# UCSD-Comp-Imaging/Nerf-Simple

Hardware: AMD Instinct MI355X
Metric: ray-samples/sec at 800x800x128 (higher is better)
Workload: dtype f16

## Files before the change

### nerf-simple_amd/csrc/mlp_bf16_16.hip

```cpp
#include "composite_device.h"

using namespace nerf_layout;

#ifdef NERF_HALF
typedef _Float16 elem_t;
#define NERF_MFMA __builtin_amdgcn_mfma_f32_16x16x32_f16
#define NERF_KERNEL nerf_mlp_f16_16_kernel
#define NERF_LAUNCH nerf_amd_launch_mlp_f16_16
#else
typedef __bf16 elem_t;
#define NERF_MFMA __builtin_amdgcn_mfma_f32_16x16x32_bf16
#define NERF_KERNEL nerf_mlp_bf16_16_kernel
#define NERF_LAUNCH nerf_amd_launch_mlp_bf16_16
#endif
#include "mlp16_chain.h"

namespace {

#ifdef NERF_HALF
constexpr bool FOLD = true;
#else
constexpr bool FOLD = false;
#endif
struct MlpPlan {
    static constexpr int LAYERS = NUM_LAYERS;
    static constexpr bool SAVE = !FOLD;
    static constexpr int tpc(int L) { return L == 0 ? 8 : 4; }
    static constexpr int mt(int L) { return FOLD ? fold_mt(L) : b16_mt(L); }
    static constexpr int layer_off_kib(int L) { return FOLD ? fold_layer_off_kib(L) : b16_layer_off_kib(L); }
    static constexpr int bias_off(int L) { return FOLD ? fold_bias_off(L) : b16_bias_off(L); }
};
static_assert(NUM_CHUNKS<MlpPlan> == (FOLD ? 34 : 38) && plan_fits<MlpPlan>(), "chunks per tile / weight buffer, parity");

constexpr int LDS_POSD = LDS_CHAIN_END;
constexpr int LDS_POSX = LDS_POSD + WAVES * NCB * 1024;
constexpr int LDS_TOTAL = LDS_POSX + WAVES * NCB * 2048;
constexpr int RING_PTS = 1024;
constexpr int LDS_RING_RAW = LDS_TOTAL;
constexpr int LDS_RING_T = LDS_RING_RAW + RING_PTS * 16;
constexpr int LDS_TOTAL_COMP = LDS_RING_T + RING_PTS * 4;
constexpr int COMP_MAX_N = RING_PTS - TILE_PTS;
static_assert(COMP_MAX_N == FUSED_RENDER_MAX_N, "api.hip routes by this limit");
static_assert(LDS_TOTAL_COMP <= 160 * 1024, "LDS budget");
static_assert((RING_PTS & (RING_PTS - 1)) == 0 && RING_PTS % TILE_PTS == 0, "ring indexing");

static_assert(ACT_TILE_PTS == TILE_PTS && MASK_TILE_PTS == TILE_PTS, "activation blocks and mask tiles are the kernel's tiles");

struct State {
    using Plan = MlpPlan;
    ex8 X[NCB][8], Y[NCB][8];
    f32x4 pend[NCB][2];
    float sigma[NCB], rgb[NCB][3];
    bool bad;
    unsigned posd_off[NCB];
    char* acts;
    long long P;
    long long tile;
    int loff[NCB];
    unsigned mb[NCB][2];
    float amax[4];
    long long mask_tile;
    long long p_end;
    unsigned ring_q0;
    WFrag* wf;
};

template <bool RAYS, int SAVE, bool COMP>
__device__ __forceinline__ void stage_inputs(const Ctx& c, const MlpArgs& a, long long tile_base, State& st) {
    const int col = c.lane & 15, g = c.lane >> 4;
    float u_mine = 0.f;
    bool dev_rng = false;
    long long b0 = 0;
    int r0 = 0;
    if constexpr (RAYS) {
        b0 = tile_base / a.N;
        r0 = (int)(tile_base - b0 * a.N);
    }
    const long long p_end = COMP ? st.p_end : a.P;
    const int last_local = (int)(p_end - 1 - tile_base);
    constexpr bool RAY_POSD = RAYS && !SAVE;
    if constexpr (RAY_POSD) {
        const int top = last_local < TILE_PTS - 1 ? last_local : TILE_PTS - 1;
        const int nrays = (int)(split_point(b0, r0, top, a.N).b - b0) + 1;
        for (int idx = threadIdx.x; idx < nrays * 32; idx += WAVES * 64) {
            const int ray = idx >> 5, slot = idx & 31, gg = slot >> 3, sl = slot & 7;
            const float* rp = a.rays + (b0 + ray) * 6 + 3;
            const float dx = rp[0], dy = rp[1], dz = rp[2];
            const float nrm = norm3(dx, dy, dz);
            float val = 0.f;
            if (sl < 6) {
                const int cd = sl >> 1;
                const float dc = __fdiv_rn(cd == 0 ? dx : cd == 1 ? dy : dz, nrm);
                val = enc_lane(to_revolutions(dc), 2 * gg + (sl & 1));
            } else if (sl == 6 && gg < 3) {
                val = __fdiv_rn(gg == 0 ? dx : gg == 1 ? dy : dz, nrm);
            }
            lds_store<elem_t>(LDS_POSD + ray * 64 + slot * 2, 0, (elem_t)val);
        }
    }
    if constexpr (RAYS && NCB == 2) {
        dev_rng = (a.flags & NERF_FLAG_DEVICE_RNG) && !(a.flags & NERF_FLAG_TS_GIVEN);
        if (dev_rng) {
            int lm = c.wave * 32 + (c.lane & 31);
            if (lm > last_local) lm = last_local;
            u_mine = device_rng_uniform(a, split_point(b0, r0, lm, a.N));
        }
    }
#pragma unroll
    for (int cb = 0; cb < NCB; ++cb) {
        long long p = tile_base + c.wave * (16 * NCB) + cb * 16 + col;
        const bool valid = p < p_end;
        st.loff[cb] = valid ? block_lane_offset(g, c.wave * (16 * NCB) + cb * 16 + col) : LOFF_INVALID;
        if constexpr (SAVE == 2) {
            if (cb == 0)
                st.loff[0] = tile_base + c.wave * 32 + 16 * (c.lane >> 5) + col < p_end ? f8_lane_offset(c.lane, c.wave) : LOFF_INVALID;
        }
        if (!valid) p = p_end - 1;
        PointIn pt;
        st.posd_off[cb] = c.b_posd + cb * 1024;
        if constexpr (RAYS) {
            const float u_cb = (NCB == 2) ? __shfl(u_mine, cb * 16 + col) : 0.f;
            int lp = c.wave * (16 * NCB) + cb * 16 + col;
            if (lp > last_local) lp = last_local;
            if (SAVE && a.pts) {
                pt = fetch_point_pts(a, p);
            } else {
                const RaySample rs = split_point(b0, r0, lp, a.N);
                if constexpr (RAY_POSD) st.posd_off[cb] = LDS_POSD + (unsigned)(rs.b - b0) * 64 + g * 16;
                pt = fetch_point_rays<!RAY_POSD>(a, p, rs, u_cb, dev_rng);
                if constexpr (COMP) {
                    if (valid && g == 0)
                        lds_store<float>(((st.ring_q0 + c.wave * (16 * NCB) + cb * 16 + col) & (RING_PTS - 1)) * 4, LDS_RING_T, pt.t);
                }
                if (valid && g == 0 && a.ts_out) a.ts_out[p] = pt.t;
            }
        } else {
            pt = fetch_point_pts(a, p);
        }
        {
            const float xyz[3] = {pt.x, pt.y, pt.z};
            float v[16];
#pragma unroll
            for (int cd = 0; cd < 3; ++cd) {
                const TwoF q = to_revolutions(xyz[cd]);
#pragma unroll
                for (int jj = 0; jj < 5; ++jj) v[cd * 5 + jj] = enc_lane(q, 5 * g + jj);
            }
            v[15] = g == 0 ? pt.x : g == 1 ? pt.y : g == 2 ? pt.z : 0.f;
#pragma unroll
            for (int e = 0; e < 2; ++e) {
                u32x4 r;
#pragma unroll
                for (int i = 0; i < 4; ++i) r[i] = pack2<false>(v[8 * e + 2 * i], v[8 * e + 2 * i + 1]);
                lds_store<u32x4>(c.b_posx, cb * 2048 + e * 1024, r);
            }
        }
        if constexpr (!RAY_POSD) {
            const float dd[3] = {pt.d1, pt.d2, pt.d3};
            float v[8];
#pragma unroll
            for (int cd = 0; cd < 3; ++cd) {
                const TwoF q = to_revolutions(dd[cd]);
#pragma unroll
                for (int jj = 0; jj < 2; ++jj) v[cd * 2 + jj] = enc_lane(q, 2 * g + jj);
            }
            v[6] = g == 0 ? pt.d1 : g == 1 ? pt.d2 : g == 2 ? pt.d3 : 0.f;
            v[7] = 0.f;
            u32x4 r;
#pragma unroll
            for (int i = 0; i < 4; ++i) r[i] = pack2<false>(v[2 * i], v[2 * i + 1]);
            lds_store<u32x4>(c.b_posd, cb * 1024, r);
        }
    }
}

template <bool RAYS, int SAVE, bool COMP>
__device__ __forceinline__ void run_tile(const Ctx& c, const MlpArgs& a, long long tile_base, State& st) {
    stage_inputs<RAYS, SAVE, COMP>(c, a, tile_base, st);
    run_layer<0, SAVE>(c, st, st.X, st.X);
    run_layer<1, SAVE>(c, st, st.X, st.Y);
    run_layer<2, SAVE>(c, st, st.Y, st.X);
    run_layer<3, SAVE>(c, st, st.X, st.Y);
    run_layer<4, SAVE>(c, st, st.Y, st.X);
    run_layer<5, SAVE>(c, st, st.X, st.Y);
    run_layer<6, SAVE>(c, st, st.Y, st.X);
    run_layer<7, SAVE>(c, st, st.X, st.Y);
    ex8 (&c_in)[NCB][8] = FOLD ? st.Y : st.X;
    ex8 (&c_out)[NCB][8] = FOLD ? st.X : st.Y;
    run_layer<8, SAVE>(c, st, st.Y, st.X);
    run_layer<9, SAVE>(c, st, c_in, c_out);
    run_layer<10, SAVE>(c, st, c_out, c_in);
    epilogue_piece<10, 0>(0, st.pend, st.X, st);
    for (int cb_ = 1; cb_ < NCB; ++cb_) epilogue_piece<10, 0>(4 * cb_, st.pend, st.X, st);
}

__device__ __forceinline__ bool finite4(float x, float y, float z, float w) {
    return __builtin_fabsf(x) + __builtin_fabsf(y) + __builtin_fabsf(z) + __builtin_fabsf(w) < __builtin_inff();
}

struct RingSamples {
    unsigned q0;
    __device__ __forceinline__ float t(int i) const {
        return lds_load<float>(((q0 + (unsigned)i) & (RING_PTS - 1)) * 4, LDS_RING_T);
    }
    __device__ __forceinline__ f32x4 c(int i) const {
        return lds_load<f32x4>(((q0 + (unsigned)i) & (RING_PTS - 1)) * 16, LDS_RING_RAW);
    }
};

template <bool RAYS, int SAVE, bool COMP>
__device__ __forceinline__ void kernel_body(const MlpArgs& a, long long ntiles) {
    static_assert(!COMP || (RAYS && !SAVE), "the fused render is the rays-mode inference kernel");
    using P = MlpPlan;
    Ctx c;
    c.wave = __builtin_amdgcn_readfirstlane(threadIdx.x >> 6);
    c.lane = threadIdx.x & 63;
    const char* img = reinterpret_cast<const char*>(a.packed);
    c.wrsrc = __builtin_amdgcn_make_buffer_rsrc(const_cast<char*>(img), 0, (int)B16_IMAGE_BYTES, 0x00020000);
    c.wave_goff = c.wave * 1024;
    c.lane16 = c.lane * 16;
#pragma unroll
    for (int p = 0; p < 2; ++p) {
        c.b_wread[p] = LDS_W0 + p * LDS_WBUF + c.lane * 16;
        c.s_wdst[p] = LDS_W0 + p * LDS_WBUF + c.wave * 1024;
    }
    c.b_bias = (c.lane >> 4) * 16;
    c.b_posx = LDS_POSX + c.wave * (NCB * 2048) + c.lane * 16;
    c.b_posd = LDS_POSD + c.wave * (NCB * 1024) + c.lane * 16;

    {
        const float* bsrc = reinterpret_cast<const float*>(img + (long long)B16_WEIGHT_KIB * 1024);
        for (int i = threadIdx.x; i < B16_BIAS_FLOATS; i += WAVES * 64)
            lds_store<float>(i * 4, LDS_BIAS, bsrc[i]);
        Stage<P, NUM_CHUNKS<P> - 1>::issue(c);
    }
    asm volatile("s_waitcnt vmcnt(0)" ::: "memory");
    __syncthreads();
    WFrag wf;
    {
        constexpr int F0 = chunk_tiles<P>(0) * (layer_desc(0).chain_k / 32 + layer_desc(0).extra_slots / 32);
#pragma unroll
        for (int f = 0; f < 4 && f < F0; ++f) wf.a[f] = lds_load<ex8>(c.b_wread[0], f * 1024);
        wf.bias0 = lds_load<f32x4>(c.b_bias, LDS_BIAS + P::bias_off(0) * 4);
    }

    if constexpr (!COMP) {
        for (long long tile = blockIdx.x; tile < ntiles; tile += gridDim.x) {
            const long long tile_base = tile * TILE_PTS;
            asm volatile("" : "+s"(c.wave_goff));
            State st;
            st.wf = &wf;
            st.acts = reinterpret_cast<char*>(a.acts);
            st.P = a.P;
            st.mask_tile = SAVE == 2 ? f8_mask_offset_bytes(0, tile, 0, a.P) : mask_offset_bytes(0, tile, 0, a.P);
            st.tile = tile;
            st.bad = false;
            run_tile<RAYS, SAVE, false>(c, a, tile_base, st);
            bool bad = st.bad;
            if (c.lane < 16) {
#pragma unroll
                for (int cb = 0; cb < NCB; ++cb) {
                    const long long p = tile_base + c.wave * (16 * NCB) + cb * 16 + c.lane;
                    if (p < a.P) {
                        const f32x4 o = {st.rgb[cb][0], st.rgb[cb][1], st.rgb[cb][2], st.sigma[cb]};
                        *reinterpret_cast<f32x4*>(a.raw + p * 4) = o;
                        bad |= !finite4(o[0], o[1], o[2], o[3]);
                    }
                }
            }
            flag_nonfinite(c, bad);
        }
    } else {
        const long long B = a.P / a.N;
        const long long r_lo = (long long)blockIdx.x * B / gridDim.x, r_hi = ((long long)blockIdx.x + 1) * B / gridDim.x;
        const long long range_base = r_lo * a.N;
        const int n_pts = (int)((r_hi - r_lo) * a.N);
        const nerf_composite::RayOut out{a.rgb, a.disp, a.alpha, a.acc, a.w, a.pixels};
        int next_ray = 0, n_complete = 0;
        for (int q_tile = 0; q_tile < n_pts; q_tile += TILE_PTS) {
            const long long tile_base = range_base + q_tile;
            asm volatile("" : "+s"(c.wave_goff));
            State st;
            st.wf = &wf;
            st.acts = nullptr;
            st.P = a.P;
            st.mask_tile = 0;
            st.tile = 0;
            st.p_end = range_base + n_pts;
            st.ring_q0 = (unsigned)q_tile & (RING_PTS - 1);
            st.bad = false;
            run_tile<true, false, true>(c, a, tile_base, st);
            bool bad = st.bad;
            if (c.lane < 16) {
#pragma unroll
                for (int cb = 0; cb < NCB; ++cb) {
                    const int local = c.wave * (16 * NCB) + cb * 16 + c.lane;
                    if (q_tile + local < n_pts) {
                        const f32x4 o = {st.rgb[cb][0], st.rgb[cb][1], st.rgb[cb][2], st.sigma[cb]};
                        lds_store<f32x4>(((st.ring_q0 + local) & (RING_PTS - 1)) * 16, LDS_RING_RAW, o);
                        bad |= !finite4(o[0], o[1], o[2], o[3]);
                    }
                }
            }
            flag_nonfinite(c, bad);
            asm volatile("s_waitcnt lgkmcnt(0)" ::: "memory");
            __builtin_amdgcn_s_barrier();
            asm volatile("" ::: "memory");
            const int done_q = q_tile + TILE_PTS < n_pts ? q_tile + TILE_PTS : n_pts;
            while ((n_complete + 1) * a.N <= done_q) ++n_complete;
            if (n_complete - next_ray >= WAVES || done_q + TILE_PTS - next_ray * a.N > RING_PTS || done_q == n_pts) {
                for (int ray = next_ray + c.wave; ray < n_complete; ray += WAVES) {
                    const long long gray = r_lo + ray;
                    const float* d = a.rays + gray * 6 + 3;
                    const float dnorm = nerf_composite::unit_dir_norm(d[0], d[1], d[2], true);
                    const RingSamples src{(unsigned)(ray * a.N) & (RING_PTS - 1)};
                    nerf_composite::composite_ray(src, a.N, c.lane, dnorm, gray, out);
                }
                next_ray = n_complete;
                asm volatile("s_waitcnt lgkmcnt(0)" ::: "memory");
                __builtin_amdgcn_s_barrier();
                asm volatile("" ::: "memory");
            }
        }
    }
}

template <bool RAYS, bool SAVE, bool COMP>
__global__ __launch_bounds__(WAVES * 64, WAVES / 4) void NERF_KERNEL(MlpArgs a, long long ntiles) {
    extern __shared__ __attribute__((aligned(16))) char smem[];
    (void)smem;
    kernel_body<RAYS, SAVE ? 1 : 0, COMP>(a, ntiles);
}
#ifndef NERF_HALF
__global__ __launch_bounds__(WAVES * 64, WAVES / 4) void nerf_mlp_train_e4m3_kernel(MlpArgs a, long long ntiles) {
    extern __shared__ __attribute__((aligned(16))) char smem[];
    (void)smem;
    kernel_body<true, 2, false>(a, ntiles);
}
#endif

}

extern "C" int NERF_LAUNCH(const MlpArgs* args, int rays_mode, hipStream_t stream) {
    (void)hipGetLastError();
    MlpArgs a = *args;
    if (a.P <= 0) return 0;
    const long long ntiles = (a.P + TILE_PTS - 1) / TILE_PTS;
    const int cus = device_cus();
    const long long grid = ntiles < cus ? ntiles : cus;
    hipError_t e = hipSuccess;
    const bool comp = a.rgb || a.disp || a.acc || a.alpha || a.w || a.pixels;
    if (comp) {
        if (!rays_mode || a.acts || a.N > COMP_MAX_N || a.P / grid + a.N >= (1ll << 31)) return -2;
        auto kern = NERF_KERNEL<true, false, true>;
        e = allow_dynamic_lds(reinterpret_cast<const void*>(kern), LDS_TOTAL_COMP);
        if (e != hipSuccess) return (int)e;
        hipLaunchKernelGGL(kern, dim3((unsigned)grid), dim3(WAVES * 64), LDS_TOTAL_COMP, stream, a, ntiles);
        return (int)hipGetLastError();
    }
#ifdef NERF_HALF
    if (a.acts) return -2;
    auto kern = rays_mode ? NERF_KERNEL<true, false, false> : NERF_KERNEL<false, false, false>;
#else
    if (a.acts && !rays_mode) return -2;
    if ((a.flags & NERF_FLAG_STORE_E4M3) && !a.acts) return -2;
    auto kern = a.acts ? ((a.flags & NERF_FLAG_STORE_E4M3) ? nerf_mlp_train_e4m3_kernel : NERF_KERNEL<true, true, false>)
                       : (rays_mode ? NERF_KERNEL<true, false, false> : NERF_KERNEL<false, false, false>);
#endif
    e = allow_dynamic_lds(reinterpret_cast<const void*>(kern), LDS_TOTAL);
    if (e != hipSuccess) return (int)e;
    hipLaunchKernelGGL(kern, dim3((unsigned)grid), dim3(WAVES * 64), LDS_TOTAL, stream, a, ntiles);
    return (int)hipGetLastError();
}
```

### nerf-simple_amd/csrc/nerf_device.h

```cpp
#pragma once
#include <hip/hip_runtime.h>
#include <stdint.h>
#include <atomic>
#include "nerf_layout.h"

typedef __bf16 bf16x8 __attribute__((ext_vector_type(8)));
typedef __bf16 bf16x2 __attribute__((ext_vector_type(2)));
typedef short s16x2 __attribute__((ext_vector_type(2)));
typedef unsigned short u16x2 __attribute__((ext_vector_type(2)));
typedef float f32x2 __attribute__((ext_vector_type(2)));
typedef float f32x4 __attribute__((ext_vector_type(4)));
typedef float f32x16 __attribute__((ext_vector_type(16)));
typedef unsigned u32x4 __attribute__((ext_vector_type(4)));

#define NERF_FLAG_TS_GIVEN 1u
#define NERF_FLAG_DEVICE_RNG 2u
#define NERF_FLAG_SEED_IN_MEMORY 4u
#define NERF_FLAG_STORE_E4M3 8u

struct MlpArgs {
    const float* pts;
    const float* rays;
    const float* u;
    const float* tbins;
    const void* packed;
    float* raw;
    float* ts_out;
    void* acts;
    long long P;
    long long ray_id0;
    unsigned long long seed;
    int N;
    unsigned flags;
    float* rgb;
    float* disp;
    float* alpha;
    float* acc;
    float* w;
    float* pixels;
};

struct DensityArgs {
    const float* pts;
    long long stride;
    const void* packed;
    float* sigma;
    long long P;
    long long ny, nz;
    float lo[3], step[3];
};

constexpr int NERF_MAX_DEVICES = 64;
inline int device_cus() {
    static int cache[NERF_MAX_DEVICES] = {};
    int dev = 0;
    if (hipGetDevice(&dev) != hipSuccess || dev < 0 || dev >= NERF_MAX_DEVICES) return 256;
    if (cache[dev] == 0) {
        int cus = 256;
        if (hipDeviceGetAttribute(&cus, hipDeviceAttributeMultiprocessorCount, dev) != hipSuccess || cus <= 0) cus = 256;
        cache[dev] = cus;
    }
    return cache[dev];
}
inline hipError_t allow_dynamic_lds(const void* kernel, int bytes) {
    struct Slot { const void* kernel; int dev; };
    static Slot slots[128];
    static std::atomic<int> used{0};
    int dev = 0;
    if (hipGetDevice(&dev) != hipSuccess) dev = -1;
    const int n = used.load(std::memory_order_acquire);
    for (int i = 0; i < n && i < 128; ++i)
        if (slots[i].kernel == kernel && slots[i].dev == dev) return hipSuccess;
    const hipError_t e = hipFuncSetAttribute(kernel, hipFuncAttributeMaxDynamicSharedMemorySize, bytes);
    if (e == hipSuccess && dev >= 0) {
        const int i = used.load(std::memory_order_relaxed);
        if (i < 128) {
            slots[i] = Slot{kernel, dev};
            used.store(i + 1, std::memory_order_release);
        }
    }
    return e;
}

constexpr int LOFF_INVALID = 0x40000000;
__host__ __device__ constexpr int swapped_chunk(int g) { return (g & 1) * 2 + (g >> 1); }
__host__ __device__ constexpr int block_lane_offset(int g, int local) { return swapped_chunk(g) * 4096 + local * 16; }

template <int AUX = 0>
__device__ __forceinline__ void store_granule(__amdgpu_buffer_rsrc_t rs, int voffset, int soffset, u32x4 w) {
    const auto s0 = __builtin_amdgcn_permlane16_swap(w[0], w[2], false, false);
    const auto s1 = __builtin_amdgcn_permlane16_swap(w[1], w[3], false, false);
    const unsigned o0 = s0[0], o1 = s1[0], o2 = s0[1], o3 = s1[1];
    __builtin_amdgcn_raw_buffer_store_b128(u32x4{o0, o1, o2, o3}, rs, voffset, soffset, AUX);
    asm volatile("s_nop 1" ::"v"(o0), "v"(o1), "v"(o2), "v"(o3) : "memory");
}

template <bool ABS>
__device__ __forceinline__ float f8_absmax(float running, float v0, float v1) {
    float r;
    if constexpr (ABS) asm("v_max3_f32 %0, %1, |%2|, |%3|" : "=v"(r) : "v"(running), "v"(v0), "v"(v1));
    else asm("v_max3_f32 %0, %1, %2, %3" : "=v"(r) : "v"(running), "v"(v0), "v"(v1));
    return r;
}
__device__ __forceinline__ int f8_wave_max_exponent(float m) {
    int r;
    asm volatile("s_nop 1\n\t"
                 "v_max_f32_dpp %1, %1, %1 quad_perm:[1,0,3,2] row_mask:0xf bank_mask:0xf\n\ts_nop 1\n\t"
                 "v_max_f32_dpp %1, %1, %1 quad_perm:[2,3,0,1] row_mask:0xf bank_mask:0xf\n\ts_nop 1\n\t"
                 "v_max_f32_dpp %1, %1, %1 row_half_mirror row_mask:0xf bank_mask:0xf\n\ts_nop 1\n\t"
                 "v_max_f32_dpp %1, %1, %1 row_mirror row_mask:0xf bank_mask:0xf\n\ts_nop 1\n\t"
                 "v_max_f32_dpp %1, %1, %1 row_bcast:15 row_mask:0xa bank_mask:0xf\n\ts_nop 1\n\t"
                 "v_max_f32_dpp %1, %1, %1 row_bcast:31 row_mask:0xc bank_mask:0xf\n\ts_nop 1\n\t"
                 "v_readlane_b32 %0, %1, 63"
                 : "=s"(r), "+v"(m));
    return (r >> 23) & 0xff;
}
__device__ __forceinline__ unsigned f8_cvt4(unsigned lo, unsigned hi, float scale) {
    unsigned r;
    asm("v_cvt_scalef32_pk_fp8_bf16 %0, %1, %3\n\tv_cvt_scalef32_pk_fp8_bf16 %0, %2, %3 op_sel:[0,0,1]"
        : "=&v"(r) : "v"(lo), "v"(hi), "s"(scale));
    return r;
}
__host__ __device__ constexpr int f8_lane_offset(int lane, int wave) {
    return ((lane >> 4) & 1) * 4096 + (wave * 32 + 16 * (lane >> 5) + (lane & 15)) * 16;
}
template <int AUX = 0>
__device__ __forceinline__ void store_fragment_f8(__amdgpu_buffer_rsrc_t rs_data, int voff, int soff_data, u32x4 w0, u32x4 w1,
                                                  float scale) {
    const unsigned a0 = f8_cvt4(w0[0], w0[1], scale), b0 = f8_cvt4(w0[2], w0[3], scale);
    unsigned a1 = f8_cvt4(w1[0], w1[1], scale), b1 = f8_cvt4(w1[2], w1[3], scale);
    asm volatile("s_nop 1" : "+v"(a1), "+v"(b1));
    const auto x0 = __builtin_amdgcn_permlane32_swap(a0, a1, false, false);
    const auto x1 = __builtin_amdgcn_permlane32_swap(b0, b1, false, false);
    const auto y0 = __builtin_amdgcn_permlane16_swap(x0[0], x1[0], false, false);
    const auto y1 = __builtin_amdgcn_permlane16_swap(x0[1], x1[1], false, false);
    const unsigned o0 = y0[0], o1 = y0[1], o2 = y1[0], o3 = y1[1];
#if defined(F8_TIMING) && F8_TIMING == 2
    asm volatile("" ::"v"(o0), "v"(o1), "v"(o2), "v"(o3));
#else
    __builtin_amdgcn_raw_buffer_store_b128(u32x4{o0, o1, o2, o3}, rs_data, voff, soff_data,
#if defined(F8_TIMING) && F8_TIMING == 3
                                           0);
#else
                                           AUX);
#endif
    asm volatile("s_nop 1" ::"v"(o0), "v"(o1), "v"(o2), "v"(o3) : "memory");
#endif
}
constexpr int F8_GROUP = 4;
template <int AUX = 0>
__device__ __forceinline__ void store_group_f8(__amdgpu_buffer_rsrc_t rs_data, int voff, int soff_data,
                                               __amdgpu_buffer_rsrc_t rs_scale, int lane, int scale_byte,
                                               const u32x4 (&w0)[F8_GROUP], const u32x4 (&w1)[F8_GROUP], float amax) {
#if defined(F8_TIMING) && F8_TIMING == 1
    const int e = (__builtin_bit_cast(int, amax) >> 23) & 0xff;
#else
    const int e = f8_wave_max_exponent(amax);
#endif
    const int sb = e > 8 ? e - 7 : 1;
    const float scale = __builtin_bit_cast(float, sb << 23);
#pragma unroll
    for (int k = 0; k < F8_GROUP; ++k) store_fragment_f8<AUX>(rs_data, voff, soff_data + k * 8192, w0[k], w1[k], scale);
#if !(defined(F8_TIMING) && F8_TIMING == 2)
    __builtin_amdgcn_raw_buffer_store_b32((unsigned)sb * 0x01010101u, rs_scale, lane == 0 ? scale_byte : LOFF_INVALID, 0, 0);
#endif
}

template <int N>
__device__ __forceinline__ void chunk_barrier() {
    asm volatile("s_waitcnt vmcnt(%0)" ::"n"(N) : "memory");
    __builtin_amdgcn_s_barrier();
    asm volatile("" ::: "memory");
}

__device__ __forceinline__ void wave_lds_fence() {
    __builtin_amdgcn_s_waitcnt(0xc07f);
    __builtin_amdgcn_wave_barrier();
}

typedef __attribute__((address_space(3))) char lds_char;
typedef __attribute__((address_space(3))) void lds_void;
template <class T>
__device__ __forceinline__ T lds_load(unsigned base, int imm) {
    return *reinterpret_cast<const __attribute__((address_space(3))) T*>(reinterpret_cast<lds_char*>(0) + base + imm);
}
template <class T>
__device__ __forceinline__ void lds_store(unsigned base, int imm, const T& v) {
    *reinterpret_cast<__attribute__((address_space(3))) T*>(reinterpret_cast<lds_char*>(0) + base + imm) = v;
}

template <class C, int NEXT, int KIB, int OFF_KIB, int WAVES>
struct ChunkDma {
    static constexpr int PIECES = (KIB + WAVES - 1) / WAVES;
    static constexpr int SRC_OFF = OFF_KIB * 1024;
    static __device__ __forceinline__ void issue_piece(const C& c, int p) {
        __builtin_amdgcn_raw_ptr_buffer_load_lds(
            c.wrsrc, reinterpret_cast<lds_void*>(reinterpret_cast<lds_char*>(0) + c.s_wdst[NEXT & 1] + p * (WAVES * 1024)), 16,
            c.lane16, c.wave_goff + (SRC_OFF + p * WAVES * 1024), 0, 0);
    }
    static __device__ __forceinline__ void issue(const C& c) {
#pragma unroll
        for (int p = 0; p < PIECES; ++p) issue_piece(c, p);
    }
};

__device__ __forceinline__ unsigned philox_word(unsigned long long seed, unsigned long long ctr) {
    unsigned c0 = (unsigned)ctr, c1 = (unsigned)(ctr >> 32), c2 = 0x6e657266u, c3 = 0x616d6421u;
    unsigned k0 = (unsigned)seed, k1 = (unsigned)(seed >> 32);
#pragma unroll
    for (int r = 0; r < 10; ++r) {
        const unsigned long long p0 = 0xD2511F53ull * c0, p1 = 0xCD9E8D57ull * c2;
        const unsigned n0 = (unsigned)(p1 >> 32) ^ c1 ^ k0, n2 = (unsigned)(p0 >> 32) ^ c3 ^ k1;
        c1 = (unsigned)p1; c3 = (unsigned)p0; c0 = n0; c2 = n2;
        k0 += 0x9E3779B9u; k1 += 0xBB67AE85u;
    }
    return c0;
}
__device__ __forceinline__ float philox_uniform(unsigned long long seed, unsigned long long ctr) {
    return (float)(philox_word(seed, ctr) >> 8) * (1.0f / 16777216.0f);
}

__device__ __forceinline__ float mul_rn(float a, float b) {
#pragma clang fp contract(off)
    return a * b;
}
__device__ __forceinline__ float add_rn(float a, float b) {
#pragma clang fp contract(off)
    return a + b;
}
__device__ __forceinline__ float sub_rn(float a, float b) {
#pragma clang fp contract(off)
    return a - b;
}
__device__ __forceinline__ float sqrt_rn(float a) { return sqrtf(a); }

__device__ __forceinline__ float norm3(float x, float y, float z) {
    return sqrt_rn(__fmaf_rn(z, z, __fmaf_rn(y, y, mul_rn(x, x))));
}

struct PointIn {
    float x, y, z, d1, d2, d3, t;
};

struct RaySample { long long b; int i; };
__device__ __forceinline__ RaySample split_point(long long b0, int r0, int local, int N) {
    const unsigned tt = (unsigned)(r0 + local);
    unsigned q = (unsigned)((float)tt * __frcp_rn((float)N));
    if ((long long)q * N > (long long)tt) --q;
    if ((long long)(q + 1) * N <= (long long)tt) ++q;
    return RaySample{b0 + q, (int)(tt - q * (unsigned)N)};
}
__device__ __forceinline__ RaySample split_point(long long p, int N) {
    const long long b = p / N;
    return RaySample{b, (int)(p - b * N)};
}

__device__ __forceinline__ unsigned long long effective_seed(const MlpArgs& a) {
    if (!(a.flags & NERF_FLAG_SEED_IN_MEMORY)) return a.seed;
    const unsigned long long v = *reinterpret_cast<const unsigned long long*>(a.u);
    const unsigned lo = __builtin_amdgcn_readfirstlane((unsigned)v), hi = __builtin_amdgcn_readfirstlane((unsigned)(v >> 32));
    return a.seed + (((unsigned long long)hi << 32) | lo);
}

__device__ __forceinline__ float device_rng_uniform(const MlpArgs& a, RaySample rs) {
    unsigned long long seed = effective_seed(a);
    asm volatile("" : "+s"(seed));
    return philox_uniform(seed, (unsigned long long)((a.ray_id0 + rs.b) * a.N + rs.i));
}

template <bool DIR = true>
__device__ __forceinline__ PointIn fetch_point_rays(const MlpArgs& a, long long p, RaySample rs, float u_pre = 0.f,
                                                    bool have_u = false) {
    PointIn r;
    const long long b = rs.b;
    const int i = rs.i;
    const float* ray = a.rays + b * 6;
    const float ox = ray[0], oy = ray[1], oz = ray[2];
    const float dx = ray[3], dy = ray[4], dz = ray[5];
    float t;
    if (a.flags & NERF_FLAG_TS_GIVEN) {
        t = __builtin_nontemporal_load(a.u + p);
    } else {
        float u;
        if (a.flags & NERF_FLAG_DEVICE_RNG)
            u = have_u ? u_pre : philox_uniform(effective_seed(a), (unsigned long long)((a.ray_id0 + b) * a.N + i));
        else
            u = __builtin_nontemporal_load(a.u + p);
        const float bin_diff = sub_rn(a.tbins[1], a.tbins[0]);
        t = add_rn(mul_rn(bin_diff, u), a.tbins[i]);
    }
    r.t = t;
    r.x = add_rn(ox, mul_rn(dx, t));
    r.y = add_rn(oy, mul_rn(dy, t));
    r.z = add_rn(oz, mul_rn(dz, t));
    if constexpr (DIR) {
        const float nrm = norm3(dx, dy, dz);
        r.d1 = __fdiv_rn(dx, nrm);
        r.d2 = __fdiv_rn(dy, nrm);
        r.d3 = __fdiv_rn(dz, nrm);
    } else {
        r.d1 = r.d2 = r.d3 = 0.f;
    }
    return r;
}

__device__ __forceinline__ PointIn fetch_point_rays(const MlpArgs& a, long long p) {
    return fetch_point_rays(a, p, split_point(p, a.N));
}

__device__ __forceinline__ PointIn fetch_point_pts(const MlpArgs& a, long long p) {
    PointIn r;
    const float* v = a.pts + p * 6;
    r.x = v[0]; r.y = v[1]; r.z = v[2];
    r.d1 = v[3]; r.d2 = v[4]; r.d3 = v[5];
    r.t = 0.f;
    return r;
}

struct TwoF { float hi, lo; };
__device__ __forceinline__ TwoF to_revolutions(float x) {
    const float C_HI = 0.15915494f;
    const float C_LO = 6.4206382e-09f;
    x = __builtin_amdgcn_fmed3f(x, -0x1p100f, 0x1p100f);
    TwoF q;
    q.hi = mul_rn(x, C_HI);
    const float err = __fmaf_rn(x, C_HI, -q.hi);
    q.lo = __fmaf_rn(x, C_LO, err);
    return q;
}
__device__ __forceinline__ float enc_lane(TwoF q, int idx) {
    const float sc = __builtin_amdgcn_ldexpf(1.0f, idx >> 1);
    const float fr = __builtin_amdgcn_fractf(q.hi * sc) + q.lo * sc + ((idx & 1) ? 0.25f : 0.f);
    return __builtin_amdgcn_sinf(fr);
}
__device__ __forceinline__ void sincos_rev_fast(TwoF q, float scale, float& s, float& c) {
    const float f = __builtin_amdgcn_fractf(q.hi * scale) + q.lo * scale;
    s = __builtin_amdgcn_sinf(f);
    c = __builtin_amdgcn_cosf(f);
}
```

Baseline: 1.390 billion.

## Stage per-tile ray records and tbins into LDS via async buffer-to-LDS DMA

```diff
diff --git a/nerf-simple_amd/csrc/mlp_bf16_16.hip b/nerf-simple_amd/csrc/mlp_bf16_16.hip
--- a/nerf-simple_amd/csrc/mlp_bf16_16.hip
+++ b/nerf-simple_amd/csrc/mlp_bf16_16.hip
@@ -45,6 +45,18 @@
 static_assert((RING_PTS & (RING_PTS - 1)) == 0 && RING_PTS % TILE_PTS == 0, "ring indexing");
 
 static_assert(ACT_TILE_PTS == TILE_PTS && MASK_TILE_PTS == TILE_PTS, "activation blocks and mask tiles are the kernel's tiles");
+
+constexpr int STAGE_MIN_N = 37;
+constexpr int STAGE_MAX_RAYS = 2 + (TILE_PTS - 2) / STAGE_MIN_N;
+constexpr int REC_RAYS = 32;
+constexpr int LDS_REC_LAND = LDS_POSD + STAGE_MAX_RAYS * 64;
+constexpr int LDS_DNORM = LDS_REC_LAND + 2 * 256;
+constexpr int LDS_BINDIFF = LDS_DNORM + REC_RAYS * 4;
+constexpr int LDS_TBINS = LDS_BINDIFF + 16;
+static_assert(STAGE_MAX_RAYS == 8 && 2 + (TILE_PTS - 2) / (STAGE_MIN_N - 1) > 8, "the bound: at most 8 rays touch a tile");
+static_assert(STAGE_MAX_RAYS * 6 <= 64, "one 64-float LDS-DMA instruction carries a tile's rays");
+static_assert((REC_RAYS & (REC_RAYS - 1)) == 0 && REC_RAYS >= RING_PTS / STAGE_MIN_N + 2, "every ray with samples in the ring, plus the tile's");
+static_assert(LDS_REC_LAND % 16 == 0 && LDS_TBINS % 16 == 0 && LDS_TBINS + COMP_MAX_N * 4 <= LDS_POSX, "the staged data fits the direction region");
 
 struct State {
     using Plan = MlpPlan;
@@ -63,7 +75,17 @@
     long long p_end;
     unsigned ring_q0;
     WFrag* wf;
+    bool staged;
+    long long r_lo;
+    int wg_rays;
 };
+
+__device__ __forceinline__ void issue_ray_dma(const MlpArgs& a, long long r_lo, int wg_rays, int half, int first_ray, int lane) {
+    const __amdgpu_buffer_rsrc_t rs = __builtin_amdgcn_make_buffer_rsrc(const_cast<float*>(a.rays) + r_lo * 6, 0, wg_rays * 24, 0x00020000);
+    const unsigned dst = __builtin_amdgcn_readfirstlane(LDS_REC_LAND + half * 256);
+    __builtin_amdgcn_raw_ptr_buffer_load_lds(rs, reinterpret_cast<lds_void*>(reinterpret_cast<lds_char*>(0) + dst), 4, lane * 4,
+                                             __builtin_amdgcn_readfirstlane(first_ray * 24), 0, 0);
+}
 
 template <bool RAYS, int SAVE, bool COMP>
 __device__ __forceinline__ void stage_inputs(const Ctx& c, const MlpArgs& a, long long tile_base, State& st) {
@@ -78,14 +100,57 @@
     }
     const long long p_end = COMP ? st.p_end : a.P;
     const int last_local = (int)(p_end - 1 - tile_base);
+    bool staged = false;
+    unsigned base = 0, land = 0;
+    int ray0 = 0, half = 0;
+    float u_mem[NCB] = {};
+    if constexpr (COMP) {
+        static_assert(NCB == 2, "the staged path takes the device draw from the shuffle below");
+        staged = st.staged;
+        if (staged) {
+            if ((a.flags & NERF_FLAG_TS_GIVEN) || !(a.flags & NERF_FLAG_DEVICE_RNG)) {
+#pragma unroll
+                for (int cb = 0; cb < NCB; ++cb) {
+                    long long p = tile_base + c.wave * (16 * NCB) + cb * 16 + col;
+                    if (p >= p_end) p = p_end - 1;
+                    u_mem[cb] = __builtin_nontemporal_load(a.u + p);
+                }
+            }
+            half = (int)(st.ring_q0 / TILE_PTS) & 1;
+            ray0 = (int)(b0 - st.r_lo);
+            base = LDS_REC_LAND;
+            asm volatile("" : "+v"(base));
+            land = base + half * 256;
+        }
+    }
     constexpr bool RAY_POSD = RAYS && !SAVE;
     if constexpr (RAY_POSD) {
         const int top = last_local < TILE_PTS - 1 ? last_local : TILE_PTS - 1;
         const int nrays = (int)(split_point(b0, r0, top, a.N).b - b0) + 1;
+        if constexpr (COMP) {
+            const int next0 = (int)(split_point(b0, r0, TILE_PTS, a.N).b - b0);
+            if (staged && c.wave == WAVES - 1 && last_local >= TILE_PTS)
+                issue_ray_dma(a, st.r_lo, st.wg_rays, half ^ 1, ray0 + next0, c.lane);
+            if (staged && c.wave == WAVES - 1 && c.lane < nrays && (c.lane > 0 || r0 == 0)) {
+                int ln = c.lane;
+                asm volatile("" : "+v"(ln));
+                const unsigned ra = land + ln * 24;
+                const float dn = nerf_composite::unit_dir_norm(lds_load<float>(ra, 12), lds_load<float>(ra, 16), lds_load<float>(ra, 20), true);
+                lds_store<float>(base + ((unsigned)(ray0 + ln) & (REC_RAYS - 1)) * 4, LDS_DNORM - LDS_REC_LAND, dn);
+            }
+        }
         for (int idx = threadIdx.x; idx < nrays * 32; idx += WAVES * 64) {
             const int ray = idx >> 5, slot = idx & 31, gg = slot >> 3, sl = slot & 7;
-            const float* rp = a.rays + (b0 + ray) * 6 + 3;
-            const float dx = rp[0], dy = rp[1], dz = rp[2];
+            float dx, dy, dz;
+            if (staged) {
+                int rl = ray;
+                asm volatile("" : "+v"(rl));
+                const unsigned ra = land + rl * 24;
+                dx = lds_load<float>(ra, 12); dy = lds_load<float>(ra, 16); dz = lds_load<float>(ra, 20);
+            } else {
+                const float* rp = a.rays + (b0 + ray) * 6 + 3;
+                dx = rp[0]; dy = rp[1]; dz = rp[2];
+            }
             const float nrm = norm3(dx, dy, dz);
             float val = 0.f;
             if (sl < 6) {
@@ -127,7 +192,17 @@
             } else {
                 const RaySample rs = split_point(b0, r0, lp, a.N);
                 if constexpr (RAY_POSD) st.posd_off[cb] = LDS_POSD + (unsigned)(rs.b - b0) * 64 + g * 16;
-                pt = fetch_point_rays<!RAY_POSD>(a, p, rs, u_cb, dev_rng);
+                if (staged) {
+                    const unsigned ra = land + (unsigned)(rs.b - b0) * 24;
+                    float tt = u_mem[cb];
+                    if (!(a.flags & NERF_FLAG_TS_GIVEN))
+                        tt = sample_position(lds_load<float>(base, LDS_BINDIFF - LDS_REC_LAND), dev_rng ? u_cb : u_mem[cb],
+                                             lds_load<float>(base + (unsigned)rs.i * 4, LDS_TBINS - LDS_REC_LAND));
+                    pt = point_on_ray(lds_load<float>(ra, 0), lds_load<float>(ra, 4), lds_load<float>(ra, 8), lds_load<float>(ra, 12),
+                                      lds_load<float>(ra, 16), lds_load<float>(ra, 20), tt);
+                } else {
+                    pt = fetch_point_rays<!RAY_POSD>(a, p, rs, u_cb, dev_rng);
+                }
                 if constexpr (COMP) {
                     if (valid && g == 0)
                         lds_store<float>(((st.ring_q0 + c.wave * (16 * NCB) + cb * 16 + col) & (RING_PTS - 1)) * 4, LDS_RING_T, pt.t);
@@ -228,10 +303,30 @@
     c.b_posx = LDS_POSX + c.wave * (NCB * 2048) + c.lane * 16;
     c.b_posd = LDS_POSD + c.wave * (NCB * 1024) + c.lane * 16;
 
+    long long r_lo = 0;
+    int wg_rays = 0;
+    bool staged = false;
+    if constexpr (COMP) {
+        const long long B = a.P / a.N;
+        const long long lo = (long long)blockIdx.x * B / gridDim.x, hi = ((long long)blockIdx.x + 1) * B / gridDim.x;
+        r_lo = (long long)(((unsigned long long)__builtin_amdgcn_readfirstlane((unsigned)((unsigned long long)lo >> 32)) << 32) |
+                           __builtin_amdgcn_readfirstlane((unsigned)lo));
+        wg_rays = __builtin_amdgcn_readfirstlane((int)(hi - lo));
+        staged = a.N >= STAGE_MIN_N;
+    }
     {
         const float* bsrc = reinterpret_cast<const float*>(img + (long long)B16_WEIGHT_KIB * 1024);
         for (int i = threadIdx.x; i < B16_BIAS_FLOATS; i += WAVES * 64)
             lds_store<float>(i * 4, LDS_BIAS, bsrc[i]);
+        if constexpr (COMP) {
+            if (staged) {
+                if (!(a.flags & NERF_FLAG_TS_GIVEN)) {
+                    for (int i = threadIdx.x; i < a.N; i += WAVES * 64) lds_store<float>(i * 4, LDS_TBINS, a.tbins[i]);
+                    if (threadIdx.x == 0) lds_store<float>(0, LDS_BINDIFF, sub_rn(a.tbins[1], a.tbins[0]));
+                }
+                if (c.wave == WAVES - 1) issue_ray_dma(a, r_lo, wg_rays, 0, 0, c.lane);
+            }
+        }
         Stage<P, NUM_CHUNKS<P> - 1>::issue(c);
     }
     asm volatile("s_waitcnt vmcnt(0)" ::: "memory");
@@ -271,10 +366,8 @@
             flag_nonfinite(c, bad);
         }
     } else {
-        const long long B = a.P / a.N;
-        const long long r_lo = (long long)blockIdx.x * B / gridDim.x, r_hi = ((long long)blockIdx.x + 1) * B / gridDim.x;
         const long long range_base = r_lo * a.N;
-        const int n_pts = (int)((r_hi - r_lo) * a.N);
+        const int n_pts = wg_rays * a.N;
         const nerf_composite::RayOut out{a.rgb, a.disp, a.alpha, a.acc, a.w, a.pixels};
         int next_ray = 0, n_complete = 0;
         for (int q_tile = 0; q_tile < n_pts; q_tile += TILE_PTS) {
@@ -289,6 +382,9 @@
             st.p_end = range_base + n_pts;
             st.ring_q0 = (unsigned)q_tile & (RING_PTS - 1);
             st.bad = false;
+            st.staged = staged;
+            st.r_lo = r_lo;
+            st.wg_rays = wg_rays;
             run_tile<true, false, true>(c, a, tile_base, st);
             bool bad = st.bad;
             if (c.lane < 16) {
@@ -311,8 +407,13 @@
             if (n_complete - next_ray >= WAVES || done_q + TILE_PTS - next_ray * a.N > RING_PTS || done_q == n_pts) {
                 for (int ray = next_ray + c.wave; ray < n_complete; ray += WAVES) {
                     const long long gray = r_lo + ray;
-                    const float* d = a.rays + gray * 6 + 3;
-                    const float dnorm = nerf_composite::unit_dir_norm(d[0], d[1], d[2], true);
+                    float dnorm;
+                    if (staged) {
+                        dnorm = lds_load<float>(((unsigned)ray & (REC_RAYS - 1)) * 4, LDS_DNORM);
+                    } else {
+                        const float* d = a.rays + gray * 6 + 3;
+                        dnorm = nerf_composite::unit_dir_norm(d[0], d[1], d[2], true);
+                    }
                     const RingSamples src{(unsigned)(ray * a.N) & (RING_PTS - 1)};
                     nerf_composite::composite_ray(src, a.N, c.lane, dnorm, gray, out);
                 }
diff --git a/nerf-simple_amd/csrc/nerf_device.h b/nerf-simple_amd/csrc/nerf_device.h
--- a/nerf-simple_amd/csrc/nerf_device.h
+++ b/nerf-simple_amd/csrc/nerf_device.h
@@ -308,6 +308,19 @@
     return fetch_point_rays(a, p, split_point(p, a.N));
 }
 
+__device__ __forceinline__ float sample_position(float bin_diff, float u, float tbin) {
+    return add_rn(mul_rn(bin_diff, u), tbin);
+}
+__device__ __forceinline__ PointIn point_on_ray(float ox, float oy, float oz, float dx, float dy, float dz, float t) {
+    PointIn r;
+    r.t = t;
+    r.x = add_rn(ox, mul_rn(dx, t));
+    r.y = add_rn(oy, mul_rn(dy, t));
+    r.z = add_rn(oz, mul_rn(dz, t));
+    r.d1 = r.d2 = r.d3 = 0.f;
+    return r;
+}
+
 __device__ __forceinline__ PointIn fetch_point_pts(const MlpArgs& a, long long p) {
     PointIn r;
     const float* v = a.pts + p * 6;
```

After: 1.386 billion. About the same (-0.3%).
